# zhangyi-3/UCDIR

Measured on AMD Instinct MI355X. Metric: restored images/sec at 50-step p_sample_loop, 256x256 SID, higher is better.
Workload: dtype bf16

## Files before the change

ucdir_amd/csrc/engine.hip:

```cpp
#include <hip/hip_runtime.h>

#include <cmath>
#include <cstdio>
#include <cstring>
#include <map>
#include <mutex>
#include <set>
#include <array>
#include <atomic>
#include <memory>
#include <string>
#include <vector>

#include "../../include/ucdir_hip.h"
#include "cgemm.hip.h"
#include "conv_halo.hip.h"
#include "akgm_halo.hip.h"
#include "akgm_pre.hip.h"
#include "akgm_ws.hip.h"
#include "akgm_ws32.hip.h"
#include "akgm_ws64.hip.h"
#include "conv_ws.hip.h"
#include "conv_sk.hip.h"
#include "conv_ws128.hip.h"
#include "flash_attn2.hip.h"
#include "qkv_ws.hip.h"
#include "common.h"
#include "misc.hip.h"
#include "fewstep.hip.h"
#include "image_metrics.hip.h"
#include "pack.h"

static thread_local std::string g_err;
static int fail(const std::string& m) { g_err = m; return 1; }
#define HIPC(x)                                                                                   \
    do {                                                                                          \
        hipError_t e_ = (x);                                                                      \
        if (e_ != hipSuccess) {                                                                   \
            throw std::runtime_error(std::string(#x) + ": " + hipGetErrorString(e_));             \
        }                                                                                         \
    } while (0)
#define API_BEGIN try {
#define API_END                                                                                   \
    }                                                                                             \
    catch (const std::exception& e) { return fail(e.what()); }                                    \
    catch (...) { return fail("unknown error"); }                                                 \
    return 0;

static void require(bool c, const std::string& m) { if (!c) throw std::runtime_error(m); }

struct DevGuard {
    int prev = -1; bool changed = false;
    explicit DevGuard(int dev) {
        HIPC(hipGetDevice(&prev));
        if (prev != dev) { HIPC(hipSetDevice(dev)); changed = true; }
    }
    ~DevGuard() { if (changed) (void)hipSetDevice(prev); }
};

struct DevPool {
    std::vector<void*> ptrs;
    int64_t bytes = 0;
    void* alloc(size_t n, bool zero = true) {
        void* p = nullptr;
        if (n == 0) n = 16;
        HIPC(hipMalloc(&p, n));
        if (zero) HIPC(hipMemset(p, 0, n));
        ptrs.push_back(p); bytes += (int64_t)n;
        return p;
    }
    template <typename T> T* upload(const std::vector<T>& v) {
        T* p = (T*)alloc(v.size() * sizeof(T), false);
        if (!v.empty()) HIPC(hipMemcpy(p, v.data(), v.size() * sizeof(T), hipMemcpyHostToDevice));
        return p;
    }
    static constexpr size_t STAT_CAP = 1 << 21;
    stat_t* stat_slab = nullptr; size_t stat_used = 0;
    stat_t* alloc_stats(int B) {
        if (!stat_slab) stat_slab = (stat_t*)alloc(STAT_CAP * sizeof(stat_t), true);
        const size_t n = (size_t)2 * UCDIR_STAT_SLOTS * B;
        if (stat_used + n > STAT_CAP) throw std::runtime_error("DevPool: statistics slab exhausted");
        stat_t* p = stat_slab + stat_used; stat_used += n;
        return p;
    }
    void zero_stats(hipStream_t st) { if (stat_used) HIPC(hipMemsetAsync(stat_slab, 0, stat_used * sizeof(stat_t), st)); }
    void release() { for (void* p : ptrs) (void)hipFree(p); ptrs.clear(); bytes = 0; stat_slab = nullptr; stat_used = 0; }
    ~DevPool() { release(); }
};

struct ConvW {
    bf16_t* A = nullptr; float* bias = nullptr; float* Tb = nullptr; float* Tg = nullptr;
    int rows_pad = 0, Kpad = 0, ntaps = 0, cin = 0, cout = 0, TM = 128; bool fold = false;
    bf16_t* Aup = nullptr; int Kup = 0;
    bf16_t* A10 = nullptr; float* bias_res = nullptr;
    bf16_t* Aws = nullptr;
    bf16_t* Aws128 = nullptr;
    bf16_t* Aqkv = nullptr;
    bf16_t* Atile = nullptr;
    bf16_t* Ask[2] = {nullptr, nullptr}; bf16_t* Ask_up[2] = {nullptr, nullptr};
    long long sk_up_stride[2] = {0, 0};
    bf16_t* Ask1x1 = nullptr;
};
struct AkgmW {
    bf16_t* A = nullptr; float* bias = nullptr; float* Tb = nullptr; float* Tg = nullptr;
    float* Tbb = nullptr;
    bf16_t* Apre = nullptr;
    bf16_t* Aws32 = nullptr;
    bf16_t* Aws64 = nullptr;
    int C = 0, cg = 0, Kpad = 0;
};

static int pick_tm(int cout) { return cout >= 128 ? 128 : 64; }

static ConvW upload_conv(DevPool& pool, const float* w, const float* bias, const float* gamma, const float* beta,
                         int cout, int cin, int ks) {
    ConvW W;
    W.TM = pick_tm(cout);
    PackedConv P = pack_conv(w, bias, gamma, beta, cout, cin, ks, W.TM);
    W.A = pool.upload(P.A); W.bias = pool.upload(P.bias);
    W.fold = gamma != nullptr;
    if (W.fold) { W.Tb = pool.upload(P.Tb); W.Tg = pool.upload(P.Tg); }
    W.rows_pad = P.rows_pad; W.Kpad = P.Kpad; W.ntaps = P.ntaps; W.cin = cin; W.cout = cout;
    if (ks == 3 && cin == 64 && cout == 64 && P.Kpad == 576) W.Aws = pool.upload(pack_conv_ws(P));
    if (ks == 3 && cin % 32 == 0 && P.Kpad == 9 * cin && P.rows_pad % W.TM == 0) W.Atile = pool.upload(pack_conv_tiled(P, W.TM));
    if (ks == 3 && cin % 32 == 0 && P.Kpad == 9 * cin && cout % 128 == 0) {
        W.Ask[0] = pool.upload(pack_conv_sk(P.A, 1, P.rows_pad, P.Kpad, cin, 9, 1));
        if (cout % 256 == 0) W.Ask[1] = pool.upload(pack_conv_sk(P.A, 1, P.rows_pad, P.Kpad, cin, 9, 2));
    }
    if (ks == 1 && cin % 32 == 0 && P.Kpad == cin && cout % 128 == 0 && gamma == nullptr) W.Ask1x1 = pool.upload(pack_conv_sk(P.A, 1, P.rows_pad, P.Kpad, cin, 1, 1));
    if (ks == 1 && cout == 3 * cin && gamma != nullptr && (cin == 256 || cin == 512) && P.Kpad == cin && P.rows_pad >= cout) W.Aqkv = pool.upload(pack_qkv_ws(P, cin));
    return W;
}
static void upload_upconv(DevPool& pool, ConvW& W, const float* w, const float* bias) {
    PackedConv P = pack_upconv(w, bias, W.cout, W.cin, W.TM);
    W.Aup = pool.upload(P.A); W.Kup = P.Kpad;
    for (int mw = 1; mw <= 2; ++mw)
        if (W.cin % 32 == 0 && W.cout % (128 * mw) == 0) {
            std::vector<bf16_t> img = pack_conv_sk(P.A, 4, P.rows_pad, P.Kpad, W.cin, 4, mw);
            W.sk_up_stride[mw - 1] = (long long)((img.size() - (size_t)4 * 4 * mw * 2 * 512) / 4);
            W.Ask_up[mw - 1] = pool.upload(img);
        }
}
static AkgmW upload_akgm(DevPool& pool, const float* wsp, const float* bsp, const float* gamma, const float* beta, int C) {
    PackedAkgm P = pack_akgm(wsp, bsp, gamma, beta, C, 0);
    AkgmW W;
    W.A = pool.upload(P.A); W.bias = pool.upload(P.bias); W.Tb = pool.upload(P.Tb); W.Tg = pool.upload(P.Tg);
    W.C = C; W.cg = P.cg; W.Kpad = P.Kpad;
    {
        std::vector<float> tbb(P.Tb.size());
// ... 11 lines not shown
struct Profiler {
    bool on = false;
    std::vector<ProfEntry> entries;
    std::vector<hipEvent_t> pool; size_t used = 0;
    hipEvent_t get() {
        if (used == pool.size()) { hipEvent_t e; HIPC(hipEventCreate(&e)); pool.push_back(e); }
        return pool[used++];
    }
    ~Profiler() { for (auto e : pool) (void)hipEventDestroy(e); }
};
static Profiler g_prof;

template <int TM, int EPI, int MODE>
static void launch_one(const GemmP& p, dim3 grid, size_t lds, hipStream_t st) {
    hipLaunchKernelGGL((cgemm_kernel<TM, EPI, MODE>), grid, dim3(CG_THREADS), lds, st, p);
}

template <typename K> static void set_lds_attr(K* k, int bytes, bool abs0 = false) {
    HIPC(hipFuncSetAttribute((const void*)k, hipFuncAttributeMaxDynamicSharedMemorySize, bytes));
    if (abs0) {
        hipFuncAttributes fa;
        HIPC(hipFuncGetAttributes(&fa, (const void*)k));
        require(fa.sharedSizeBytes == 0, "a kernel with absolute LDS addressing has static __shared__ memory: its dynamic smem[] no longer starts at offset 0");
    }
}
template <int TM> static void set_cgemm_attrs() {
    set_lds_attr(cgemm_kernel<TM, EPI_STD, MODE_S1>, 100 * 1024, true); set_lds_attr(cgemm_kernel<TM, EPI_STD, MODE_DOWN>, 100 * 1024, true);
    set_lds_attr(cgemm_kernel<TM, EPI_STD, MODE_UP>, 100 * 1024, true); set_lds_attr(cgemm_kernel<TM, EPI_STD, MODE_PLAIN>, 100 * 1024, true);
    set_lds_attr(cgemm_kernel<TM, EPI_STD, MODE_S1C>, 100 * 1024, true); set_lds_attr(cgemm_kernel<TM, EPI_AKGM, MODE_S1>, 100 * 1024, true);
}
#define SPLITK_MAX_WGS 512
#define SK_MAX_GRID 256
#define SCRATCH_BYTES ((size_t)2 * SK_MAX_GRID * 65536 * sizeof(float))
static std::map<int, float*> g_splitk_buf;
static std::mutex g_static_mu;
static void ensure_kernel_attrs() {
    std::lock_guard<std::mutex> lk(g_static_mu);
    static std::set<int> done;
    int dev = 0;
    HIPC(hipGetDevice(&dev));
    if (done.count(dev)) return;
    set_cgemm_attrs<64>(); set_cgemm_attrs<128>();
    set_lds_attr(conv3x3_halo_kernel<128, false>, hc_lds_bytes<128>());
    set_lds_attr(conv3x3_halo_kernel<64, false>, hc_lds_bytes<64>());
    set_lds_attr(conv3x3_halo_kernel<64, true>, hc_lds_bytes<64>());
    set_lds_attr(akgm_halo_stage_kernel, AH_LDS); set_lds_attr(akgm_halo_kernel<true>, AH_LDS);
    set_lds_attr(akgm_pre_kernel<8>, AkPre<8>::LDS);
    set_lds_attr(akgm_ws_kernel<8>, AkWs::LDS); set_lds_attr(akgm_ws_kernel<16>, AkWs::LDS);
    set_lds_attr(akgm_ws32_kernel<32>, AkWs32::LDS); set_lds_attr(akgm_ws32_kernel<16>, AkWs32::LDS); set_lds_attr(akgm_ws32_kernel<8>, AkWs32::LDS);
    set_lds_attr(akgm_ws64_kernel<2, 8, true>, 160 * 1024); set_lds_attr(akgm_ws64_kernel<4, 8, true>, 160 * 1024);
    set_lds_attr(qkv_ws_kernel<256>, QkvWs::LDS); set_lds_attr(qkv_ws_kernel<512>, QkvWs::LDS);
    set_lds_attr(conv_ws_kernel, CvWs::LDS);
    set_lds_attr(conv_ws128_kernel, CvWs128::LDS);
    set_lds_attr(conv_sk_kernel<2, 8, 9>, 160 * 1024); set_lds_attr(conv_sk_kernel<2, 8, 4>, 160 * 1024);
    set_lds_attr(conv_sk_kernel<1, 8, 9>, 160 * 1024); set_lds_attr(conv_sk_kernel<1, 8, 4>, 160 * 1024);
    set_lds_attr(conv_sk_kernel<1, 4, 9>, 80 * 1024, true); set_lds_attr(conv_sk_kernel<1, 4, 4>, 80 * 1024, true);

    set_lds_attr(final_conv_kernel, 160 * 1024);
    set_lds_attr(flash_attn2_kernel<1, false>, fa_lds_bytes(128), true); set_lds_attr(flash_attn2_kernel<1, true>, fa_lds_bytes(128), true);
    set_lds_attr(flash_attn2_kernel<2, false>, fa_lds_bytes(256), true); set_lds_attr(flash_attn2_kernel<2, true>, fa_lds_bytes(256), true);
    set_lds_attr(flash_attn2_kernel<3, false>, fa_lds_bytes(384), true); set_lds_attr(flash_attn2_kernel<3, true>, fa_lds_bytes(384), true);
    set_lds_attr(flash_attn2_kernel<4, false>, fa_lds_bytes(512), true); set_lds_attr(flash_attn2_kernel<4, true>, fa_lds_bytes(512), true);
    done.insert(dev);
}

static void gemm_work(const GemmP& p, int epi, double& flops, double& bytes) {
    const double cols = ((p.cols_mode == COLS_PLAIN) ? (double)p.W : (double)p.H * p.W) * (p.up_phase ? 4.0 : 1.0);
    if (epi == EPI_AKGM) {
        const double C = 8.0 * p.cg;
        flops = 2.0 * 9 * C * C * cols * p.nbatch;
        bytes = (2.0 * C * cols * 2 + C * cols * 2 + cols * 32) * p.nbatch + 9.0 * C * C * 2;
    } else {
        const double K = (double)p.ntaps * p.cg;
        flops = 2.0 * K * p.nfeat * cols * p.nbatch;
        double in_cols = cols;
        if (p.cols_mode == COLS_DOWN) in_cols = cols * 4; else if (p.cols_mode == COLS_UP) in_cols = cols / 4;
        bytes = ((double)p.cg * in_cols * 2 + (double)p.nfeat * cols * (p.out_f32 ? 4 : 2) + (p.res ? (double)p.nfeat * cols * 2 : 0)) * p.nbatch
                + (p.a_bstride ? (double)p.nfeat * K * 2 * p.nbatch : (double)p.nfeat * K * 2);
    }
}

static void launch_cgemm_impl(const GemmP& p, int TM, int epi, hipStream_t st);
static void launch_cgemm(const GemmP& p, int TM, int epi, hipStream_t st) {
    if (!g_prof.on) { launch_cgemm_impl(p, TM, epi, st); return; }
    ProfEntry e;
    int mode = p.cols_mode; if (mode == COLS_S1 && p.in_compact) mode = MODE_S1C;
    e.key = (TM == 128 ? 100 : 0) + (epi == EPI_AKGM ? 10 : 0) + (epi == EPI_AKGM ? 0 : mode);
    gemm_work(p, epi, e.flops, e.bytes);
    e.dH = p.H; e.dW = p.W; e.dCin = p.cg * p.ntaps; e.dCout = p.nfeat;
    e.e0 = g_prof.get(); e.e1 = g_prof.get();
    HIPC(hipEventRecord(e.e0, st));
    launch_cgemm_impl(p, TM, epi, st);
    HIPC(hipEventRecord(e.e1, st));
    g_prof.entries.push_back(e);
}

static void launch_cgemm_impl(const GemmP& p0, int TM, int epi, hipStream_t st) {
    GemmP p = p0;
#ifdef UCDIR_TIMING
    static unsigned long long* cgdbg = nullptr;
    if (!cgdbg) HIPC(hipMalloc((void**)&cgdbg, 64 * 8));
    HIPC(hipMemsetAsync(cgdbg, 0, 64 * 8, st));
    p.dbg = cgdbg;
    struct Pr { unsigned long long* d; hipStream_t s; int mode, TM, nk; ~Pr() {
        unsigned long long h[64]; (void)hipStreamSynchronize(s); (void)hipMemcpy(h, d, sizeof(h), hipMemcpyDeviceToHost);
        const int n = (int)h[63]; fprintf(stderr, "CGEMM TIMING mode=%d TM=%d nk=%d n=%d:", mode, TM, nk, n);
// ... 364 lines not shown
    if (!dbgbuf) HIPC(hipMalloc((void**)&dbgbuf, 256 * 8));
    HIPC(hipMemset(dbgbuf, 0, 256 * 8));
    p.dbg = dbgbuf;
#endif
    int tm_run = w.TM;
    if (halo && tm_run == 128 && p.nbatch * p.tiles * p.rowtiles < 256) {
        tm_run = 64; p.rowtiles = w.rows_pad / 64;
    }
    static const bool fuse_res = !getenv("UCDIR_NO_FUSED_RES");
    bool did_res = false;
    if (halo && !upph && tm_run == 64 && w.TM == 64 && w.A10 && res_out && fuse_res) {
        p.A = w.A10; p.a_ld = 10 * cin; p.res_fused = 1; p.bias2 = w.bias_res;
        p.out2 = res_out->p; p.out2_bstride = res_out->bstride(); p.out2_ld = res_out->C;
        did_res = true;
    }
    const bool dual = did_res;
    static const bool use_atile = !getenv("UCDIR_NO_ATILE");
    if (use_atile && halo && !upph && !did_res && tm_run == w.TM && w.Atile && w.ntaps == 9) p.A_tiled = w.Atile;
    static const bool use_cws128 = !getenv("UCDIR_NO_CONV_WS128");
    if (use_cws128 && did_res && w.Aws128 && cin == 128 && x0.C == 64 && x1 && x1->C == 64 && !res && !p.out_nchw && y.H % 8 == 0 && y.W % 16 == 0 &&
        y.C == 64 && (g_persist_grid > 0 || (long long)y.B * (y.H / 8) * (y.W / 16) >= 4LL * num_cus())) {
        p.A = w.Aws128; p.alt_A = w.Aws128 + (size_t)2 * 72 * 2 * 32 * 8;
        p.th = 8; p.tw = 16; p.tiles_x = y.W / 16; p.tiles_y = y.H / 8;
        const int ntiles = y.B * p.tiles_x * p.tiles_y, ncu = num_cus();
        const int grid = ntiles < ncu ? ntiles : ncu;
#ifdef UCDIR_TIMING
        {
            static unsigned long long* dbgbuf = nullptr;
            if (!dbgbuf) HIPC(hipMalloc((void**)&dbgbuf, 256 * 8));
            HIPC(hipMemset(dbgbuf, 0, 256 * 8));
            p.dbg = dbgbuf;
            hipLaunchKernelGGL(conv_ws128_kernel, dim3(grid), dim3(CvWs128::THREADS), CvWs128::LDS, st, p);
            unsigned long long h[256];
            HIPC(hipStreamSynchronize(st));
            HIPC(hipMemcpy(h, dbgbuf, sizeof(h), hipMemcpyDeviceToHost));
            const int n = (int)h[255];
            fprintf(stderr, "CONV_WS128 TIMING n=%d:", n);
            for (int i = 1; i < n && i < 255; ++i) fprintf(stderr, " %llu", h[i] - h[i - 1]);
            fprintf(stderr, "\n");
            return did_res;
        }
#endif
        if (g_prof.on) {
            ProfEntry e; e.key = 24; gemm_work(p, EPI_STD, e.flops, e.bytes);
            { const double cols = (double)p.H * p.W * p.nbatch; e.flops += 2.0 * p.cg * p.nfeat * cols; e.bytes += 2.0 * p.cg * p.nfeat + 2.0 * p.nfeat * cols; }
            e.dH = p.H; e.dW = p.W; e.dCin = p.cg; e.dCout = p.nfeat;
            e.e0 = g_prof.get(); e.e1 = g_prof.get();
            HIPC(hipEventRecord(e.e0, st));
            hipLaunchKernelGGL(conv_ws128_kernel, dim3(grid), dim3(CvWs128::THREADS), CvWs128::LDS, st, p);
            HIPC(hipEventRecord(e.e1, st));
            g_prof.entries.push_back(e);
        } else {
            hipLaunchKernelGGL(conv_ws128_kernel, dim3(grid), dim3(CvWs128::THREADS), CvWs128::LDS, st, p);
        }
        HIPC(hipGetLastError());
        return did_res;
    }
    if (halo && !did_res && !p.out_nchw && w.cout % 8 == 0) {
        const int taps = upph ? 4 : 9, tps = 256 / tm_run;
        const int ks = choose_ksplit(p.nbatch * p.tiles * p.rowtiles, cin / HC_BK, (taps + tps - 1) / tps,
                                     (double)y.B * y.H * y.W * w.cout);
        if (ks > 1) { p.ksplit = ks; p.partial = splitk_scratch(); }
    }
    static const bool tail_res = !getenv("UCDIR_NO_TAIL_RES");
    if (halo && !upph && !did_res && res_out && wres && tail_res && !p.out_nchw && wres->ntaps == 1 &&
        wres->rows_pad >= p.rowtiles * tm_run) {
        p.alt_blocks = p.nbatch * p.tiles * p.rowtiles;
        p.alt_A = wres->A; p.alt_a_ld = wres->Kpad; p.bias2 = wres->bias;
        p.out2 = res_out->p; p.out2_bstride = res_out->bstride(); p.out2_ld = res_out->C;
        did_res = true;
    }
    static const bool use_cws = !getenv("UCDIR_NO_CONV_WS");
    if (use_cws && halo && !upph && !did_res && !dual && w.Aws && !x1 && !res && !p.out_nchw && p.ksplit <= 1 && !p.alt_blocks &&
        y.H % 16 == 0 && y.W % 16 == 0 && x0.C == 64 && y.C == 64 &&
        (g_persist_grid > 0 || (long long)y.B * (y.H / 16) * (y.W / 16) >= 4LL * num_cus())) {
        p.A = w.Aws; p.th = 16; p.tw = 16; p.tiles_x = y.W / 16; p.tiles_y = y.H / 16;
        const int ntiles = y.B * p.tiles_x * p.tiles_y, ncu = num_cus();
        const int grid = ntiles < ncu ? ntiles : ncu;
#ifdef UCDIR_TIMING
        {
            static unsigned long long* dbgbuf = nullptr;
            if (!dbgbuf) HIPC(hipMalloc((void**)&dbgbuf, 512 * 8));
            HIPC(hipMemset(dbgbuf, 0, 512 * 8));
            p.dbg = dbgbuf;
            hipLaunchKernelGGL(conv_ws_kernel, dim3(grid), dim3(HC_THREADS), CvWs::LDS, st, p);
            unsigned long long h[512];
            HIPC(hipStreamSynchronize(st));
            HIPC(hipMemcpy(h, dbgbuf, sizeof(h), hipMemcpyDeviceToHost));
            for (int w = 0; w < 2; ++w) {
                const int n = (int)h[w * 256 + 255];
                fprintf(stderr, "CONV_WS TIMING %s n=%d:", w ? "late" : "early", n);
                for (int i = 1; i < n && i < 255; ++i) fprintf(stderr, " %llu", h[w * 256 + i] - h[w * 256 + i - 1]);
                fprintf(stderr, "\n");
            }
            return did_res;
        }
#endif
        if (g_prof.on) {
            ProfEntry e; e.key = 23; gemm_work(p, EPI_STD, e.flops, e.bytes);
            e.dH = p.H; e.dW = p.W; e.dCin = p.cg; e.dCout = p.nfeat;
            e.e0 = g_prof.get(); e.e1 = g_prof.get();
            HIPC(hipEventRecord(e.e0, st));
            hipLaunchKernelGGL(conv_ws_kernel, dim3(grid), dim3(HC_THREADS), CvWs::LDS, st, p);
            HIPC(hipEventRecord(e.e1, st));
            g_prof.entries.push_back(e);
        } else {
// ... 479 lines not shown
}

static const std::vector<float>& W_(ucdir_ctx* c, const std::string& name, size_t expect) {
    auto it = c->host.find(name);
    require(it != c->host.end(), "missing weight: " + name);
    require(it->second.v.size() == expect, "weight " + name + " has wrong size");
    return it->second.v;
}

static void finalize_weights(ucdir_ctx* c) {
    const auto& cfg = c->cfg;
    const int inner = cfg.inner_channel;
    c->wpool.release();
    c->lw.assign(c->layers.size(), LayerW());
    c->mlp_w1 = c->wpool.upload(W_(c, "noise_level_mlp.1.weight", (size_t)4 * inner * inner));
    c->mlp_b1 = c->wpool.upload(W_(c, "noise_level_mlp.1.bias", (size_t)4 * inner));
    c->mlp_w2 = c->wpool.upload(W_(c, "noise_level_mlp.3.weight", (size_t)4 * inner * inner));
    c->mlp_b2 = c->wpool.upload(W_(c, "noise_level_mlp.3.bias", (size_t)inner));
    std::vector<float> tw;
    int nb = 0;
    for (size_t li = 0; li < c->layers.size(); ++li) {
        const LayerDesc& d = c->layers[li];
        LayerW& w = c->lw[li];
        if (d.kind == "stem") {
            const auto& sw = W_(c, d.name + ".weight", (size_t)d.cout * d.cin * 9);
            require(d.cin == 6, "stem expects in_channel == 6 (cat[cond, x_t])");
            std::vector<float> t((size_t)54 * d.cout);
            for (int o = 0; o < d.cout; ++o) for (int ci = 0; ci < 6; ++ci) for (int k = 0; k < 9; ++k)
                t[(size_t)(k * 6 + ci) * d.cout + o] = sw[((size_t)o * 6 + ci) * 9 + k];
            require(d.cout % 64 == 0, "stem: inner_channel must be a multiple of 64");
            w.stem_w = c->wpool.upload(pack_stem_frags(t, W_(c, d.name + ".bias", (size_t)d.cout), 6, d.cout));
        } else if (d.kind == "down" || d.kind == "up") {
            w.conv = upload_conv(c->wpool, W_(c, d.name + ".conv.weight", (size_t)d.cout * d.cin * 9).data(),
                                 W_(c, d.name + ".conv.bias", d.cout).data(), nullptr, nullptr, d.cout, d.cin, 3);
            if (d.kind == "up") upload_upconv(c->wpool, w.conv, W_(c, d.name + ".conv.weight", (size_t)d.cout * d.cin * 9).data(),
                                              W_(c, d.name + ".conv.bias", d.cout).data());
        } else {
            const std::string r = d.name + ".res_block.";
            w.block_index = nb++;
            w.conv = upload_conv(c->wpool, W_(c, r + "conv1.weight", (size_t)d.cout * d.cin * 9).data(),
                                 W_(c, r + "conv1.bias", d.cout).data(), W_(c, r + "norm1.weight", d.cin).data(),
                                 W_(c, r + "norm1.bias", d.cin).data(), d.cout, d.cin, 3);
            w.has_res = d.cin != d.cout;
            if (w.has_res) {
                w.resconv = upload_conv(c->wpool, W_(c, r + "res_conv.weight", (size_t)d.cout * d.cin).data(),
                                        W_(c, r + "res_conv.bias", d.cout).data(), nullptr, nullptr, d.cout, d.cin, 1);
                if (w.conv.TM == 64 && d.cin % 64 == 0 && w.conv.Kpad == 9 * d.cin) {
                    PackedConv P = pack_conv(W_(c, r + "conv1.weight", (size_t)d.cout * d.cin * 9).data(), nullptr,
                                             W_(c, r + "norm1.weight", d.cin).data(), W_(c, r + "norm1.bias", d.cin).data(),
                                             d.cout, d.cin, 3, 64);
                    const std::vector<bf16_t> a10 = pack_conv_res10(P, W_(c, r + "res_conv.weight", (size_t)d.cout * d.cin).data());
                    w.conv.A10 = c->wpool.upload(a10);
                    if (d.cin == 128 && d.cout == 64) w.conv.Aws128 = c->wpool.upload(pack_conv_ws128(a10));
                    w.conv.bias_res = w.resconv.bias;
                }
            }
            w.sp = upload_akgm(c->wpool, W_(c, r + "spdyconv.weight", (size_t)8 * d.cout * (d.cout / 8) * 9).data(),
                               W_(c, r + "spdyconv.bias", (size_t)8 * d.cout).data(), W_(c, r + "norm2.weight", d.cout).data(),
                               W_(c, r + "norm2.bias", d.cout).data(), d.cout);
            std::vector<float> gw;
            for (const char* s : {"conv2.0.weight", "conv2.0.bias", "conv2.2.weight", "conv2.2.bias"}) {
                const auto& v = c->host.at(r + s).v;
                gw.insert(gw.end(), v.begin(), v.end());
            }
            require(gw.size() == 48 + 16 + 576 + 8, "guide branch weights have wrong size");
            w.gw = c->wpool.upload(gw);
            for (const char* s : {"noise_func.0.weight", "noise_func.0.bias", "noise_func.2.weight", "noise_func.2.bias"}) {
                const auto& v = c->host.at(r + s).v;
                tw.insert(tw.end(), v.begin(), v.end());
            }
            if (d.attn) {
                const std::string a = d.name + ".attn.";
                const std::vector<float> wf = fold_out_into_v(W_(c, a + "qkv.weight", (size_t)3 * d.cout * d.cout).data(),
                                                              W_(c, a + "out.weight", (size_t)d.cout * d.cout).data(), d.cout);
                w.qkv = upload_conv(c->wpool, wf.data(), nullptr,
                                    W_(c, a + "norm.weight", d.cout).data(), W_(c, a + "norm.bias", d.cout).data(),
                                    3 * d.cout, d.cout, 1);
                w.outp = upload_conv(c->wpool, W_(c, a + "out.weight", (size_t)d.cout * d.cout).data(),
                                     W_(c, a + "out.bias", d.cout).data(), nullptr, nullptr, d.cout, d.cout, 1);
            }
        }
    }
    c->nblocks = nb;
    require(tw.size() == (size_t)nb * (8 * inner + 8 + 64 + 8), "time weights have wrong size");
    c->tw = c->wpool.upload(tw);
    const int fc = inner * cfg.channel_mults[0];
    c->fin_gamma = c->wpool.upload(W_(c, "final_conv.0.weight", fc));
    c->fin_beta = c->wpool.upload(W_(c, "final_conv.0.bias", fc));
    c->fin_conv = upload_conv(c->wpool, W_(c, "final_conv.3.weight", (size_t)cfg.out_channel * fc * 9).data(),
                              W_(c, "final_conv.3.bias", cfg.out_channel).data(), nullptr, nullptr, cfg.out_channel, fc, 3);
    if (cfg.out_channel <= 4 && fc % 32 == 0) {
        c->fin_w = c->wpool.upload(pack_final_frags(W_(c, "final_conv.3.weight", (size_t)cfg.out_channel * fc * 9).data(), cfg.out_channel, fc));
        c->fin_b = c->wpool.upload(W_(c, "final_conv.3.bias", cfg.out_channel));
    }
    c->host.clear();
    c->finalized = true;
}

static int level_dim(int d, int level) { return d >> level; }

struct ActPlanner {
    DevPool& pool; int B; bool reuse;
    std::map<std::array<int, 3>, std::vector<bf16_t*>> free_;
    Act get(int h, int w, int C, bool stats = true) {
        Act a; a.B = B; a.H = h; a.W = w; a.C = C;
        auto& fl = free_[{h, w, C}];
// ... 581 lines not shown
}

int32_t ucdir_op_conv(const float* x0, int32_t c0, const float* x1, int32_t c1, int32_t B, int32_t H, int32_t W,
                      const float* w_host, const float* bias_host, const float* gamma_host, const float* beta_host,
                      int32_t cout, int32_t ksize, int32_t mode, int32_t silu, const float* residual, float* y,
                      double* stats_out_host, void* stream) {
    API_BEGIN
    ensure_kernel_attrs();
    hipStream_t st = (hipStream_t)stream;
    DevPool pool;
    Act a0 = act_from_nchw(pool, x0, B, c0, H, W, st, true);
    Act a1; if (x1) a1 = act_from_nchw(pool, x1, B, c1, H, W, st, true);
    int Ho = H, Wo = W;
    if (mode == COLS_DOWN) { Ho = H / 2; Wo = W / 2; } else if (mode == COLS_UP) { Ho = 2 * H; Wo = 2 * W; }
    Act out = make_act(pool, B, Ho, Wo, cout);
    Act res; if (residual) res = act_from_nchw(pool, residual, B, cout, Ho, Wo, st, false);
    ConvW w = upload_conv(pool, w_host, bias_host, gamma_host, beta_host, cout, c0 + (x1 ? c1 : 0), ksize);
    if (mode == COLS_UP && ksize == 3) upload_upconv(pool, w, w_host, bias_host);
    run_conv(w, a0, x1 ? &a1 : nullptr, out, mode, silu, residual ? &res : nullptr, true, st);
    hipLaunchKernelGGL(act_to_nchw_kernel, dim3(2048), dim3(256), 0, st, out.p, y, B, cout, Ho, Wo);
    HIPC(hipGetLastError());
    std::vector<stat_t> sfx;
    if (stats_out_host) { sfx.resize((size_t)2 * UCDIR_STAT_SLOTS * B); HIPC(hipMemcpyAsync(sfx.data(), out.stats, sizeof(stat_t) * sfx.size(), hipMemcpyDeviceToHost, st)); }
    HIPC(hipStreamSynchronize(st));
    if (stats_out_host)
        for (int bb = 0; bb < B; ++bb)
            for (int q = 0; q < 2; ++q) {
                stat_t acc = 0;
                for (int k = 0; k < UCDIR_STAT_SLOTS; ++k) acc += sfx[((size_t)bb * UCDIR_STAT_SLOTS + k) * 2 + q];
                stats_out_host[bb * 2 + q] = (double)acc / UCDIR_STAT_SCALE;
            }
    API_END
}

int32_t ucdir_op_conv_res(const float* x0, int32_t c0, const float* x1, int32_t c1, int32_t B, int32_t H, int32_t W,
                          const float* w_host, const float* bias_host, const float* gamma_host, const float* beta_host,
                          const float* wres_host, const float* bres_host, int32_t cout, int32_t silu,
                          float* y, float* yres, double* stats_out_host, void* stream) {
    API_BEGIN
    ensure_kernel_attrs();
    hipStream_t st = (hipStream_t)stream;
    DevPool pool;
    const int cin = c0 + (x1 ? c1 : 0);
    Act a0 = act_from_nchw(pool, x0, B, c0, H, W, st, true);
    Act a1; if (x1) a1 = act_from_nchw(pool, x1, B, c1, H, W, st, true);
    Act out = make_act(pool, B, H, W, cout), rout = make_act(pool, B, H, W, cout, false);
    ConvW w = upload_conv(pool, w_host, bias_host, gamma_host, beta_host, cout, cin, 3);
    ConvW wr = upload_conv(pool, wres_host, bres_host, nullptr, nullptr, cout, cin, 1);
    if (w.TM == 64 && cin % 64 == 0 && w.Kpad == 9 * cin) {
        PackedConv P = pack_conv(w_host, nullptr, gamma_host, beta_host, cout, cin, 3, 64);
        const std::vector<bf16_t> a10 = pack_conv_res10(P, wres_host);
        w.A10 = pool.upload(a10); w.bias_res = wr.bias;
        if (cin == 128 && cout == 64) w.Aws128 = pool.upload(pack_conv_ws128(a10));
    }
    const bool did = run_conv(w, a0, x1 ? &a1 : nullptr, out, COLS_S1, silu, nullptr, true, st, nullptr, 0, 0, &rout, &wr);
    if (!did) run_conv(wr, a0, x1 ? &a1 : nullptr, rout, COLS_S1, 0, nullptr, false, st);
    hipLaunchKernelGGL(act_to_nchw_kernel, dim3(2048), dim3(256), 0, st, out.p, y, B, cout, H, W);
    hipLaunchKernelGGL(act_to_nchw_kernel, dim3(2048), dim3(256), 0, st, rout.p, yres, B, cout, H, W);
    HIPC(hipGetLastError());
    std::vector<stat_t> sfx;
    if (stats_out_host) { sfx.resize((size_t)2 * UCDIR_STAT_SLOTS * B); HIPC(hipMemcpyAsync(sfx.data(), out.stats, sizeof(stat_t) * sfx.size(), hipMemcpyDeviceToHost, st)); }
    HIPC(hipStreamSynchronize(st));
    if (stats_out_host)
        for (int bb = 0; bb < B; ++bb)
            for (int q = 0; q < 2; ++q) {
                stat_t acc = 0;
                for (int k = 0; k < UCDIR_STAT_SLOTS; ++k) acc += sfx[((size_t)bb * UCDIR_STAT_SLOTS + k) * 2 + q];
                stats_out_host[bb * 2 + q] = (double)acc / UCDIR_STAT_SCALE;
            }
    API_END
}

int32_t ucdir_op_akgm(const float* h, const float* att, const float* res, int32_t B, int32_t C, int32_t H, int32_t W,
                      const float* wsp_host, const float* bsp_host, const float* gamma_host, const float* beta_host,
                      float* y, double* stats_out_host, void* stream) {
    API_BEGIN
    ensure_kernel_attrs();
    hipStream_t st = (hipStream_t)stream;
    DevPool pool;
    Act ah = act_from_nchw(pool, h, B, C, H, W, st, true);
    Act ar = act_from_nchw(pool, res, B, C, H, W, st, false);
    Act out = make_act(pool, B, H, W, C);
    float* G = (float*)pool.alloc((size_t)B * H * W * 8 * 4);
    hipLaunchKernelGGL(nchw8_to_compact_kernel, dim3(1024), dim3(256), 0, st, att, G, B, H, W);
    std::vector<float> ones((size_t)B * 8, 1.f);
    float* attw = pool.upload(ones);
    AkgmW w = upload_akgm(pool, wsp_host, bsp_host, gamma_host, beta_host, C);
    float* tcbuf = (float*)pool.alloc((size_t)B * (9 * 8 * C + 2) * sizeof(float), false);
    run_akgm(w, ah, G, attw, ar, out, tcbuf, st);
    hipLaunchKernelGGL(act_to_nchw_kernel, dim3(2048), dim3(256), 0, st, out.p, y, B, C, H, W);
    HIPC(hipGetLastError());
    std::vector<stat_t> sfx;
    if (stats_out_host) { sfx.resize((size_t)2 * UCDIR_STAT_SLOTS * B); HIPC(hipMemcpyAsync(sfx.data(), out.stats, sizeof(stat_t) * sfx.size(), hipMemcpyDeviceToHost, st)); }
    HIPC(hipStreamSynchronize(st));
    if (stats_out_host)
        for (int bb = 0; bb < B; ++bb)
            for (int q = 0; q < 2; ++q) {
                stat_t acc = 0;
                for (int k = 0; k < UCDIR_STAT_SLOTS; ++k) acc += sfx[((size_t)bb * UCDIR_STAT_SLOTS + k) * 2 + q];
                stats_out_host[bb * 2 + q] = (double)acc / UCDIR_STAT_SCALE;
            }
    API_END
}

int32_t ucdir_op_attention(const float* x, int32_t B, int32_t C, int32_t H, int32_t W, const float* gamma_host,
                           const float* beta_host, const float* wqkv_host, const float* wout_host, const float* bout_host,
// ... 265 lines not shown
```

ucdir_amd/csrc/pack.h:

```cpp
#pragma once
#include <cmath>
#include <cstdint>
#include <vector>

#include "common.h"

struct PackedConv {
    std::vector<bf16_t> A;
    std::vector<float> bias;
    std::vector<float> Tb, Tg;
    int rows_pad = 0, Kpad = 0, ntaps = 0, cin = 0, cout = 0, ncls = 0;
};

static inline bool tap_valid(int cls, int tap) {
    const int cy = cls / 3, cx = cls % 3, ky = tap / 3, kx = tap % 3;
    if (cy == 0 && ky == 0) return false;
    if (cy == 2 && ky == 2) return false;
    if (cx == 0 && kx == 0) return false;
    if (cx == 2 && kx == 2) return false;
    return true;
}

static inline PackedConv pack_conv(const float* w, const float* bias, const float* gamma, const float* beta,
                                   int cout, int cin, int ks, int TM) {
// ... 14 lines not shown
                const float ws = fold ? wv * gamma[c] : wv;
                const bf16_t q = f2bf(ws);
                P.A[(size_t)o * P.Kpad + (size_t)t * cin + c] = q;
                if (fold) {
                    wb[(size_t)t * cout + o] += (double)wv * beta[c];
                    wg[(size_t)t * cout + o] += (double)bf2f(q);
                }
            }
    if (fold) {
        P.Tb.assign((size_t)P.ncls * cout, 0.f);
        P.Tg.assign((size_t)P.ncls * cout, 0.f);
        for (int cls = 0; cls < P.ncls; ++cls)
            for (int o = 0; o < cout; ++o) {
                double sb = 0, sg = 0;
                for (int t = 0; t < P.ntaps; ++t) {
                    const int t9 = (P.ntaps == 9) ? t : 4;
                    if (P.ncls == 9 && !tap_valid(cls, t9)) continue;
                    sb += wb[(size_t)t * cout + o]; sg += wg[(size_t)t * cout + o];
                }
                P.Tb[(size_t)cls * cout + o] = (float)sb;
                P.Tg[(size_t)cls * cout + o] = (float)sg;
            }
    }
    return P;
}

static inline std::vector<bf16_t> pack_conv_ws(const PackedConv& P) {
    std::vector<bf16_t> img((size_t)2 * 36 * 2 * 32 * 8, 0);
    for (int rw = 0; rw < 2; ++rw)
        for (int j = 0; j < 36; ++j)
            for (int hk = 0; hk < 2; ++hk)
                for (int rho = 0; rho < 32; ++rho) {
                    const int o = 32 * rw + 16 * ((rho >> 2) & 1) + (rho & 3) + 4 * (rho >> 3);
                    const int tap = j >> 2, c0 = 16 * (j & 3) + 8 * hk;
                    for (int e = 0; e < 8; ++e)
                        img[((((size_t)rw * 36 + j) * 2 + hk) * 32 + rho) * 8 + e] = P.A[(size_t)o * P.Kpad + (size_t)tap * 64 + c0 + e];
                }
    return img;
}

static inline std::vector<bf16_t> pack_conv_ws128(const std::vector<bf16_t>& A10) {
    const int K10 = 10 * 128, nj = 80;
    std::vector<bf16_t> img((size_t)2 * nj * 2 * 32 * 8, 0);
    for (int rw = 0; rw < 2; ++rw)
        for (int j = 0; j < nj; ++j)
            for (int hk = 0; hk < 2; ++hk)
                for (int rho = 0; rho < 32; ++rho) {
                    const int o = 32 * rw + 16 * ((rho >> 2) & 1) + (rho & 3) + 4 * (rho >> 3);
                    const int tap = j >> 3, c0 = 16 * (j & 7) + 8 * hk;
                    const size_t dst = j < 72 ? ((((size_t)rw * 72 + j) * 2 + hk) * 32 + rho) * 8
                                              : (size_t)2 * 72 * 2 * 32 * 8 + ((((size_t)rw * 8 + (j - 72)) * 2 + hk) * 32 + rho) * 8;
                    for (int e = 0; e < 8; ++e) img[dst + e] = A10[(size_t)o * K10 + (size_t)tap * 128 + c0 + e];
                }
    return img;
}

static inline std::vector<bf16_t> pack_conv_res10(const PackedConv& P, const float* wres) {
    const int cin = P.cin, K10 = 10 * cin;
    std::vector<bf16_t> A((size_t)P.rows_pad * K10, 0);
    for (int o = 0; o < P.rows_pad; ++o) {
        for (int k = 0; k < 9 * cin; ++k) A[(size_t)o * K10 + k] = P.A[(size_t)o * P.Kpad + k];
        if (o < P.cout)
            for (int c = 0; c < cin; ++c) A[(size_t)o * K10 + 9 * cin + c] = f2bf(wres[(size_t)o * cin + c]);
    }
    return A;
}

struct PackedAkgm {
    std::vector<bf16_t> A;
    std::vector<float> bias;
    std::vector<float> Tb, Tg;
    int C = 0, cg = 0, Kpad = 0;
};

static inline PackedAkgm pack_akgm(const float* wsp, const float* bsp, const float* gamma, const float* beta, int C,
                                   int kpad_override = 0) {
    PackedAkgm P;
    P.C = C; P.cg = C / 8;
    const int cg = P.cg;
    const bool chunked = (cg == 64) && !kpad_override;
    P.Kpad = kpad_override ? kpad_override : (chunked ? 640 : ((9 * cg + 63) / 64) * 64);
    P.A.assign((size_t)8 * C * P.Kpad, 0);
    P.bias.assign((size_t)8 * C, 0.f);
    P.Tb.assign((size_t)9 * 8 * C, 0.f);
    P.Tg.assign((size_t)9 * 8 * C, 0.f);
    for (int o = 0; o < 8 * C; ++o) P.bias[o] = bsp[o];
    for (int g = 0; g < 8; ++g)
        for (int pr = 0; pr < C; ++pr) {
            const int t32 = pr / 32, rho = pr % 32;
            const int floc = 4 * t32 + ((rho >> 4) & 1) * 2 + ((rho >> 2) & 1);
            const int s = (rho & 3) + 4 * ((rho >> 3) & 1);
            const int o = g * C + 8 * floc + s;
            bf16_t* row = &P.A[((size_t)g * C + pr) * P.Kpad];
            double wb[9] = {0}, wg[9] = {0};
            for (int ci = 0; ci < cg; ++ci) {
                const int cglob = g * cg + ci;
                for (int t = 0; t < 9; ++t) {
                    const float wv = wsp[((size_t)o * cg + ci) * 9 + t];
                    const bf16_t q = f2bf(wv * gamma[cglob]);
                    row[chunked ? (size_t)(ci / 32) * 320 + (size_t)t * 32 + (ci % 32) : (size_t)t * cg + ci] = q;
                    wb[t] += (double)wv * beta[cglob];
                    wg[t] += (double)bf2f(q);
                }
            }
            for (int cls = 0; cls < 9; ++cls) {
                double sb = 0, sg = 0;
// ... 178 lines not shown
```

Baseline: 37.00.

## Add persistent weight-stationary conv kernel for 192-to-64 residual blocks

Adds a specialized persistent weight-stationary 3x3 conv kernel for cin=192 (128+64 concatenated inputs), cout=64. It also fuses the 1x1 residual conv. Weights are held in registers, and a double-buffered halo is staged in LDS. The K dimension is split across wave pairs, and the partial sums are exchanged through LDS. It replaces the generic path for these decoder blocks. The cost is heavy register pressure from the 60 weight fragments held per lane, plus new packing code.

After: 37.25 (median of 6 runs). Within noise of the previous version (+0.7%).

```diff
diff --git a/ucdir_amd/csrc/conv_ws192.hip.h b/ucdir_amd/csrc/conv_ws192.hip.h
--- /dev/null
+++ b/ucdir_amd/csrc/conv_ws192.hip.h
@@ -0,0 +1,297 @@
+#pragma once
+#include <type_traits>
+#include "conv_ws128.hip.h"
+
+struct CvWs192 {
+    static constexpr int TH = 4, TW = 16;
+    static constexpr int PITCH = 24;
+    static constexpr int PLANE = 6 * PITCH * 128;
+    static constexpr int HALO = 3 * PLANE;
+    static constexpr int QSTEP = 2 * PITCH * 128;
+    static constexpr int OFF_X = 2 * HALO;
+    static constexpr int X_WAVE = 8 * 64 * 16;
+    static constexpr int OFF_TCS = OFF_X + 4 * X_WAVE;
+    static constexpr int OFF_B2 = OFF_TCS + 9 * 64 * 4;
+    static constexpr int OFF_SCAL = OFF_B2 + 64 * 4;
+    static constexpr int LDS = OFF_SCAL + 128;
+    static constexpr int THREADS = 256;
+    static constexpr int DEPTH = 3;
+    static constexpr int NJ = 54;
+};
+
+__global__ __launch_bounds__(CvWs192::THREADS, 1) void conv_ws192_kernel(const GemmP p) {
+    using L = CvWs192;
+    extern __shared__ __attribute__((aligned(16))) unsigned char smem[];
+    float* const tcs = reinterpret_cast<float*>(smem + L::OFF_TCS);
+    float* const b2s = reinterpret_cast<float*>(smem + L::OFF_B2);
+    float* const scal = reinterpret_cast<float*>(smem + L::OFF_SCAL);
+    const int tid = threadIdx.x, lane = tid & 63, l31 = lane & 31, hh = lane >> 5;
+    const int wave = __builtin_amdgcn_readfirstlane(tid >> 6);
+    const int rw = wave & 1, kh = wave >> 1;
+    const int prow = l31 >> 4, pcol = (l31 & 15) ^ (prow << 3);
+    int lid;
+    {
+        const int nblk = gridDim.x, bid = blockIdx.x;
+        const int q = nblk >> 3, r = nblk & 7, xcd = bid & 7;
+        lid = (xcd < r ? xcd * (q + 1) : r * (q + 1) + (xcd - r) * q) + (bid >> 3);
+    }
+#ifdef UCDIR_TIMING
+    const bool dbg_on = p.dbg && (lid == (int)gridDim.x / 2 + 3) && (lane == 0) && (wave == 1);
+    int dbg_n = 0;
+#define C9_STAMP() do { if (dbg_on && dbg_n < 250) p.dbg[dbg_n++] = __builtin_amdgcn_s_memtime(); } while (0)
+#else
+#define C9_STAMP() do {} while (0)
+#endif
+    C9_STAMP();
+    const int tps = p.tiles_x * p.tiles_y;
+    const int T = p.nbatch * tps;
+    const int t_beg = (int)((long long)lid * T / (int)gridDim.x), t_end = (int)((long long)(lid + 1) * T / (int)gridDim.x);
+    if (t_beg >= t_end) return;
+
+    bf16x8_t af[L::NJ], ra[6];
+    {
+        const bf16_t* Ab = p.A + ((((rw * 2 + kh) * (L::NJ + 6)) * 2 + hh) * 32 + l31) * 8;
+#pragma unroll
+        for (int j = 0; j < L::NJ; ++j) af[j] = *reinterpret_cast<const bf16x8_t*>(Ab + j * (2 * 32 * 8));
+#pragma unroll
+        for (int j = 0; j < 6; ++j) ra[j] = *reinterpret_cast<const bf16x8_t*>(Ab + (L::NJ + j) * (2 * 32 * 8));
+    }
+#pragma unroll
+    for (int j = 0; j < L::NJ; ++j) asm volatile("" : "+v"(af[j]));
+#pragma unroll
+    for (int j = 0; j < 6; ++j) asm volatile("" : "+v"(ra[j]));
+    if (tid < 64) b2s[tid] = p.bias2 ? p.bias2[tid] : 0.f;
+    __syncthreads();
+
+    const int nunits = wave < 2 ? 5 : 4;
+    unsigned hrel[5][3];
+#pragma unroll
+    for (int s = 0; s < 5; ++s) {
+        const int u = wave + 4 * s, r = u / 3, pl = u - 3 * r;
+        const int C = pl == 2 ? 64 : 128, chb = pl == 1 ? 64 : 0;
+#pragma unroll
+        for (int c3 = 0; c3 < 3; ++c3) {
+            const int col = c3 * 8 + (lane >> 3), gcol = col < 18 ? col : 17, hp = r * L::PITCH + col;
+            hrel[s][c3] = (unsigned)((r * p.Wp + gcol) * C + chb + (((lane & 7) ^ ((hp >> 1) & 7)) << 3)) * 2u;
+        }
+    }
+    auto issue_piece = [&](const unsigned char* h0, const unsigned char* h1, unsigned char* hd, int s, int c3) {
+        const int u = wave + 4 * s, r = u / 3, pl = u - 3 * r;
+        stage16(reinterpret_cast<const bf16_t*>((pl == 2 ? h1 : h0) + hrel[s][c3]), hd + pl * L::PLANE + (3 * r + c3) * 1024, lane);
+    };
+    unsigned ba[3][4], bb[3][2][2];
+    {
+        const int hp0 = prow * L::PITCH + pcol;
+#pragma unroll
+        for (int kx = 0; kx < 3; ++kx) {
+            const int sxh = (((hp0 + kx) >> 1) & 7) ^ hh;
+#pragma unroll
+            for (int k2 = 0; k2 < 4; ++k2) ba[kx][k2] = kh * 2 * L::PLANE + ((hp0 + kx) << 7) + (((2 * k2) ^ sxh) << 4);
+#pragma unroll
+            for (int c = 0; c < 2; ++c)
+#pragma unroll
+                for (int f = 0; f < 2; ++f)
+                    bb[kx][c][f] = L::PLANE + ((hp0 + kx) << 7) + (((2 * ((2 * kh + c) ^ (2 * f))) ^ sxh) << 4);
+        }
+    }
+    const unsigned tc_lane = L::OFF_TCS + (32 * rw + 16 * hh) * 4;
+    const unsigned b2_lane = L::OFF_B2 + (32 * rw + 16 * hh) * 4;
+    const unsigned x_put = L::OFF_X + (rw * 2 + kh) * L::X_WAVE + lane * 16;
+    const unsigned x_get = L::OFF_X + (rw * 2 + (kh ^ 1)) * L::X_WAVE + lane * 16;
+    const unsigned rel_out = (unsigned)(((2 * kh + prow + 1) * p.Wp + pcol + 1) * 64 + 32 * rw + 16 * hh) * 2;
+
+    int b, ty, tx;
+    {
+        b = t_beg / tps;
+        const int r = t_beg - b * tps;
+        ty = r / p.tiles_x; tx = r - ty * p.tiles_x;
+    }
+    auto tile_src = [&](int nb, int nty, int ntx, const unsigned char*& h0, const unsigned char*& h1) {
+        const long long pix0 = (long long)nty * L::TH * p.Wp + ntx * L::TW;
+        h0 = reinterpret_cast<const unsigned char*>(p.B0 + (long long)nb * p.b0_bstride + pix0 * 128);
+        h1 = reinterpret_cast<const unsigned char*>(p.B1 + (long long)nb * p.b1_bstride + pix0 * 64);
+    };
+    {
+        const unsigned char *h0, *h1;
+        tile_src(b, ty, tx, h0, h1);
+#pragma unroll
+        for (int s = 0; s < 5; ++s)
+            if (s < nunits)
+#pragma unroll
+                for (int c3 = 0; c3 < 3; ++c3) issue_piece(h0, h1, smem, s, c3);
+    }
+
+    int b_cur = -1;
+    float rstd_a = 1.f;
+    stat_t S1 = 0, S2 = 0;
+    const int act = p.act;
+
+#pragma unroll 1
+    for (int t = t_beg; t < t_end; ++t) {
+        const int buf = (t - t_beg) & 1;
+        const bool last = t + 1 == t_end;
+        C9_STAMP();
+        if (t == t_beg) { HC_WAIT(0); }
+        asm volatile("s_barrier" ::: "memory");
+        C9_STAMP();
+        if (b != b_cur) {
+            if (b_cur >= 0 && p.stats_out) {
+                const stat_t a = wave_sum_ll(S1), q2 = wave_sum_ll(S2);
+                if (lane == 0) stat_add_fx(p.stats_out, b_cur, a, q2);
+            }
+            S1 = 0; S2 = 0;
+            b_cur = b;
+            if (wave == 0) {
+                float mean = 0.f, rstd = 1.f;
+                if (p.fold) {
+                    long long v = 0;
+                    if (lane < 2 * UCDIR_STAT_SLOTS) {
+                        v = p.stats0[(long long)b * (2 * UCDIR_STAT_SLOTS) + lane];
+                        if (p.stats1) v += p.stats1[(long long)b * (2 * UCDIR_STAT_SLOTS) + lane];
+                    }
+#pragma unroll
+                    for (int off = 2; off < 2 * UCDIR_STAT_SLOTS; off <<= 1) v += __shfl_xor(v, off);
+                    const long long q = __shfl(v, 1);
+                    mean_rstd(stat_val(v), stat_val(q), p.inv_count, mean, rstd);
+                }
+                if (lane == 0) { scal[0] = mean; scal[1] = rstd; }
+            }
+            __syncthreads();
+            const float mean = scal[0], rstd = scal[1];
+            for (int i = tid; i < 9 * 64; i += L::THREADS) {
+                const int cls = i >> 6, f = i & 63;
+                float v = p.bias ? p.bias[f] : 0.f;
+                if (p.fold) v += p.Tb[(long long)cls * p.tab_ld + f] - mean * rstd * p.Tg[(long long)cls * p.tab_ld + f];
+                tcs[i] = v;
+            }
+            rstd_a = __builtin_bit_cast(float, __builtin_amdgcn_readfirstlane(__builtin_bit_cast(int, p.alpha * (p.fold ? rstd : 1.0f))));
+            __syncthreads();
+        }
+        int nb = b, nty = ty, ntx = tx + 1;
+        if (ntx == p.tiles_x) { ntx = 0; if (++nty == p.tiles_y) { nty = 0; ++nb; } }
+
+        if (t != t_beg) {
+            const int d = buf ? L::HALO : -L::HALO;
+#pragma unroll
+            for (int kx = 0; kx < 3; ++kx) {
+#pragma unroll
+                for (int k2 = 0; k2 < 4; ++k2) ba[kx][k2] += d;
+#pragma unroll
+                for (int c = 0; c < 2; ++c) { bb[kx][c][0] += d; bb[kx][c][1] += d; }
+            }
+        }
+
+        f32x16_t acc[2], acc2[2];
+        {
+            bf16x8_t bq[L::DEPTH + 1][2];
+            const unsigned char *h0, *h1;
+            tile_src(nb, nty, ntx, h0, h1);
+            unsigned char* const hd = smem + (buf ^ 1) * L::HALO;
+            auto read_step = [&](auto jc, bf16x8_t (&dst)[2]) {
+                constexpr int j = decltype(jc)::value;
+                constexpr int tap = j / 6, cl = j % 6, ky = tap / 3, kx = tap - 3 * ky;
+                constexpr int off = ky * (L::PITCH * 128);
+                if constexpr (cl < 4) {
+                    lds_read16_asm<off>(dst[0], ba[kx][cl ^ (ky == 1 ? 2 : 0)]);
+                    lds_read16_asm<off + L::QSTEP>(dst[1], ba[kx][cl ^ (ky == 1 ? 2 : 0)]);
+                } else {
+                    lds_read16_asm<off>(dst[0], bb[kx][cl & 1][ky == 1 ? 1 : 0]);
+                    lds_read16_asm<off + L::QSTEP>(dst[1], bb[kx][cl & 1][ky == 1 ? 1 : 0]);
+                }
+            };
+            __builtin_amdgcn_sched_barrier(0);
+            asm volatile("s_waitcnt lgkmcnt(0)" ::: "memory");
+            static_for<0, L::DEPTH>([&](auto jc) { read_step(jc, bq[decltype(jc)::value]); });
+            static_for<0, L::NJ>([&](auto jc) {
+                constexpr int j = decltype(jc)::value;
+                if constexpr (j + L::DEPTH < L::NJ)
+                    read_step(std::integral_constant<int, j + L::DEPTH>{}, bq[(j + L::DEPTH) % (L::DEPTH + 1)]);
+                if constexpr (j % 3 == 1 && j / 3 < 15) {
+                    constexpr int e = j / 3, s = e / 3, c3 = e % 3;
+                    if (!last && s < nunits) issue_piece(h0, h1, hd, s, c3);
+                }
+                constexpr int ahead = (L::NJ - 1 - j) < L::DEPTH ? (L::NJ - 1 - j) : L::DEPTH;
+                lgkm_wait_asm<2 * ahead>();
+                const f32x16_t zero = {0.f, 0.f, 0.f, 0.f, 0.f, 0.f, 0.f, 0.f, 0.f, 0.f, 0.f, 0.f, 0.f, 0.f, 0.f, 0.f};
+                const bf16x8_t* bj = bq[j % (L::DEPTH + 1)];
+                acc[0] = __builtin_amdgcn_mfma_f32_32x32x16_bf16(af[j], bj[0], j ? acc[0] : zero, 0, 0, 0);
+                acc[1] = __builtin_amdgcn_mfma_f32_32x32x16_bf16(af[j], bj[1], j ? acc[1] : zero, 0, 0, 0);
+                if constexpr (j / 6 == 4) {
+                    constexpr int cl = j % 6;
+                    acc2[0] = __builtin_amdgcn_mfma_f32_32x32x16_bf16(ra[cl], bj[0], cl ? acc2[0] : zero, 0, 0, 0);
+                    acc2[1] = __builtin_amdgcn_mfma_f32_32x32x16_bf16(ra[cl], bj[1], cl ? acc2[1] : zero, 0, 0, 0);
+                }
+            });
+            __builtin_amdgcn_sched_barrier(0);
+        }
+        C9_STAMP();
+        f32x16_t own, own2;
+        {
+            const f32x16_t give = kh ? acc[0] : acc[1], give2 = kh ? acc2[0] : acc2[1];
+            own = kh ? acc[1] : acc[0]; own2 = kh ? acc2[1] : acc2[0];
+#pragma unroll
+            for (int g = 0; g < 4; ++g) {
+                const f32x4_t v = {give[4 * g], give[4 * g + 1], give[4 * g + 2], give[4 * g + 3]};
+                const f32x4_t w = {give2[4 * g], give2[4 * g + 1], give2[4 * g + 2], give2[4 * g + 3]};
+                *reinterpret_cast<f32x4_t*>(smem + x_put + 1024 * g) = v;
+                *reinterpret_cast<f32x4_t*>(smem + x_put + 1024 * (4 + g)) = w;
+            }
+        }
+        asm volatile("s_waitcnt lgkmcnt(0)\n\ts_barrier" ::: "memory");
+        C9_STAMP();
+        const bool interior = ty > 0 && tx > 0 && ty + 1 < p.tiles_y && tx + 1 < p.tiles_x;
+        const long long tile_el = (long long)(ty * L::TH * p.Wp + tx * L::TW) * 64;
+        unsigned char* outb = reinterpret_cast<unsigned char*>(reinterpret_cast<bf16_t*>(p.out) + (long long)b * p.out_bstride + tile_el);
+        unsigned char* out2b = reinterpret_cast<unsigned char*>(p.out2 + (long long)b * p.out2_bstride + tile_el);
+        float s1 = 0.f, s2 = 0.f;
+        uint4 pk[2], pk2[2];
+        {
+            unsigned tca = tc_lane + 4 * 256;
+            if (!interior) {
+                const int r = 2 * kh + prow, c = pcol;
+                const int cy = (ty == 0 && r == 0) ? 0 : ((ty + 1 == p.tiles_y && r == L::TH - 1) ? 2 : 1);
+                const int cx = (tx == 0 && c == 0) ? 0 : ((tx + 1 == p.tiles_x && c == L::TW - 1) ? 2 : 1);
+                tca = tc_lane + (cy * 3 + cx) * 256;
+            }
+            float v[16], w[16];
+#pragma unroll
+            for (int g = 0; g < 4; ++g) {
+                const f32x4_t o4 = *reinterpret_cast<const f32x4_t*>(smem + x_get + 1024 * g);
+                const f32x4_t o24 = *reinterpret_cast<const f32x4_t*>(smem + x_get + 1024 * (4 + g));
+                const f32x4_t c4 = *reinterpret_cast<const f32x4_t*>(smem + tca + 16 * g);
+                const f32x4_t d4 = *reinterpret_cast<const f32x4_t*>(smem + b2_lane + 16 * g);
+#pragma unroll
+                for (int e = 0; e < 4; ++e) {
+                    v[4 * g + e] = fmaf(own[4 * g + e] + o4[e], rstd_a, c4[e]);
+                    w[4 * g + e] = (own2[4 * g + e] + o24[e]) + d4[e];
+                }
+            }
+            if (act == 1) {
+#pragma unroll
+                for (int i = 0; i < 16; ++i) v[i] = silu_fast(v[i]);
+            } else if (act == 2) {
+#pragma unroll
+                for (int i = 0; i < 16; ++i) v[i] = fmaxf(0.2f * v[i], v[i]);
+            }
+#pragma unroll
+            for (int i = 0; i < 16; ++i) { s1 += v[i]; s2 += v[i] * v[i]; }
+            pk[0] = pack8_bf16(v); pk[1] = pack8_bf16(v + 8);
+            pk2[0] = pack8_bf16(w); pk2[1] = pack8_bf16(w + 8);
+        }
+        C9_STAMP();
+        HC_WAIT(0);
+        *reinterpret_cast<uint4*>(outb + rel_out) = pk[0];
+        *reinterpret_cast<uint4*>(outb + rel_out + 16) = pk[1];
+        *reinterpret_cast<uint4*>(out2b + rel_out) = pk2[0];
+        *reinterpret_cast<uint4*>(out2b + rel_out + 16) = pk2[1];
+        S1 += stat_fx((double)s1); S2 += stat_fx((double)s2);
+        b = nb; ty = nty; tx = ntx;
+    }
+#ifdef UCDIR_TIMING
+    if (dbg_on) p.dbg[255] = dbg_n;
+#endif
+    if (p.stats_out) {
+        const stat_t a = wave_sum_ll(S1), q2 = wave_sum_ll(S2);
+        if (lane == 0) stat_add_fx(p.stats_out, b_cur, a, q2);
+    }
+}
diff --git a/ucdir_amd/csrc/engine.hip b/ucdir_amd/csrc/engine.hip
--- a/ucdir_amd/csrc/engine.hip
+++ b/ucdir_amd/csrc/engine.hip
@@ -23,6 +23,7 @@
 #include "conv_ws.hip.h"
 #include "conv_sk.hip.h"
 #include "conv_ws128.hip.h"
+#include "conv_ws192.hip.h"
 #include "flash_attn2.hip.h"
 #include "qkv_ws.hip.h"
 #include "common.h"
@@ -95,6 +96,7 @@
     bf16_t* A10 = nullptr; float* bias_res = nullptr;
     bf16_t* Aws = nullptr;
     bf16_t* Aws128 = nullptr;
+    bf16_t* Aws192 = nullptr;
     bf16_t* Aqkv = nullptr;
     bf16_t* Atile = nullptr;
     bf16_t* Ask[2] = {nullptr, nullptr}; bf16_t* Ask_up[2] = {nullptr, nullptr};
@@ -212,6 +214,7 @@
     set_lds_attr(qkv_ws_kernel<256>, QkvWs::LDS); set_lds_attr(qkv_ws_kernel<512>, QkvWs::LDS);
     set_lds_attr(conv_ws_kernel, CvWs::LDS);
     set_lds_attr(conv_ws128_kernel, CvWs128::LDS);
+    set_lds_attr(conv_ws192_kernel, CvWs192::LDS);
     set_lds_attr(conv_sk_kernel<2, 8, 9>, 160 * 1024); set_lds_attr(conv_sk_kernel<2, 8, 4>, 160 * 1024);
     set_lds_attr(conv_sk_kernel<1, 8, 9>, 160 * 1024); set_lds_attr(conv_sk_kernel<1, 8, 4>, 160 * 1024);
     set_lds_attr(conv_sk_kernel<1, 4, 9>, 80 * 1024, true); set_lds_attr(conv_sk_kernel<1, 4, 4>, 80 * 1024, true);
@@ -682,6 +685,45 @@
             g_prof.entries.push_back(e);
         } else {
             hipLaunchKernelGGL(conv_ws128_kernel, dim3(grid), dim3(CvWs128::THREADS), CvWs128::LDS, st, p);
+        }
+        HIPC(hipGetLastError());
+        return did_res;
+    }
+    if (use_cws128 && did_res && w.Aws192 && cin == 192 && x0.C == 128 && x1 && x1->C == 64 && !res && !p.out_nchw &&
+        y.H % CvWs192::TH == 0 && y.W % CvWs192::TW == 0 && y.C == 64 &&
+        (g_persist_grid > 0 || (long long)y.B * (y.H / CvWs192::TH) * (y.W / CvWs192::TW) >= 4LL * num_cus())) {
+        p.A = w.Aws192;
+        p.th = CvWs192::TH; p.tw = CvWs192::TW; p.tiles_x = y.W / CvWs192::TW; p.tiles_y = y.H / CvWs192::TH;
+        const int ntiles = y.B * p.tiles_x * p.tiles_y;
+        const int grid = ntiles < num_cus() ? ntiles : num_cus();
+#ifdef UCDIR_TIMING
+        {
+            static unsigned long long* dbgbuf = nullptr;
+            if (!dbgbuf) HIPC(hipMalloc((void**)&dbgbuf, 256 * 8));
+            HIPC(hipMemset(dbgbuf, 0, 256 * 8));
+            p.dbg = dbgbuf;
+            hipLaunchKernelGGL(conv_ws192_kernel, dim3(grid), dim3(CvWs192::THREADS), CvWs192::LDS, st, p);
+            unsigned long long h[256];
+            HIPC(hipStreamSynchronize(st));
+            HIPC(hipMemcpy(h, dbgbuf, sizeof(h), hipMemcpyDeviceToHost));
+            const int n = (int)h[255];
+            fprintf(stderr, "CONV_WS192 TIMING n=%d:", n);
+            for (int i = 1; i < n && i < 255; ++i) fprintf(stderr, " %llu", h[i] - h[i - 1]);
+            fprintf(stderr, "\n");
+            return did_res;
+        }
+#endif
+        if (g_prof.on) {
+            ProfEntry e; e.key = 26; gemm_work(p, EPI_STD, e.flops, e.bytes);
+            { const double cols = (double)p.H * p.W * p.nbatch; e.flops += 2.0 * p.cg * p.nfeat * cols; e.bytes += 2.0 * p.cg * p.nfeat + 2.0 * p.nfeat * cols; }
+            e.dH = p.H; e.dW = p.W; e.dCin = p.cg; e.dCout = p.nfeat;
+            e.e0 = g_prof.get(); e.e1 = g_prof.get();
+            HIPC(hipEventRecord(e.e0, st));
+            hipLaunchKernelGGL(conv_ws192_kernel, dim3(grid), dim3(CvWs192::THREADS), CvWs192::LDS, st, p);
+            HIPC(hipEventRecord(e.e1, st));
+            g_prof.entries.push_back(e);
+        } else {
+            hipLaunchKernelGGL(conv_ws192_kernel, dim3(grid), dim3(CvWs192::THREADS), CvWs192::LDS, st, p);
         }
         HIPC(hipGetLastError());
         return did_res;
@@ -1267,6 +1309,7 @@
                     const std::vector<bf16_t> a10 = pack_conv_res10(P, W_(c, r + "res_conv.weight", (size_t)d.cout * d.cin).data());
                     w.conv.A10 = c->wpool.upload(a10);
                     if (d.cin == 128 && d.cout == 64) w.conv.Aws128 = c->wpool.upload(pack_conv_ws128(a10));
+                    if (d.cin == 192 && d.cout == 64) w.conv.Aws192 = c->wpool.upload(pack_conv_ws192(a10));
                     w.conv.bias_res = w.resconv.bias;
                 }
             }
@@ -1954,6 +1997,7 @@
         const std::vector<bf16_t> a10 = pack_conv_res10(P, wres_host);
         w.A10 = pool.upload(a10); w.bias_res = wr.bias;
         if (cin == 128 && cout == 64) w.Aws128 = pool.upload(pack_conv_ws128(a10));
+        if (cin == 192 && cout == 64) w.Aws192 = pool.upload(pack_conv_ws192(a10));
     }
     const bool did = run_conv(w, a0, x1 ? &a1 : nullptr, out, COLS_S1, silu, nullptr, true, st, nullptr, 0, 0, &rout, &wr);
     if (!did) run_conv(wr, a0, x1 ? &a1 : nullptr, rout, COLS_S1, 0, nullptr, false, st);
diff --git a/ucdir_amd/csrc/pack.h b/ucdir_amd/csrc/pack.h
--- a/ucdir_amd/csrc/pack.h
+++ b/ucdir_amd/csrc/pack.h
@@ -90,6 +90,23 @@
                                               : (size_t)2 * 72 * 2 * 32 * 8 + ((((size_t)rw * 8 + (j - 72)) * 2 + hk) * 32 + rho) * 8;
                     for (int e = 0; e < 8; ++e) img[dst + e] = A10[(size_t)o * K10 + (size_t)tap * 128 + c0 + e];
                 }
+    return img;
+}
+
+static inline std::vector<bf16_t> pack_conv_ws192(const std::vector<bf16_t>& A10) {
+    const int cin = 192, K10 = 10 * cin, nj = 60;
+    std::vector<bf16_t> img((size_t)2 * 2 * nj * 2 * 32 * 8, 0);
+    for (int rw = 0; rw < 2; ++rw)
+        for (int kh = 0; kh < 2; ++kh)
+            for (int j = 0; j < nj; ++j)
+                for (int hk = 0; hk < 2; ++hk)
+                    for (int rho = 0; rho < 32; ++rho) {
+                        const int o = 32 * rw + 16 * ((rho >> 2) & 1) + (rho & 3) + 4 * (rho >> 3);
+                        const int tap = j < 54 ? j / 6 : 9, cl = j < 54 ? j % 6 : j - 54;
+                        const int c0 = (kh == 0 ? 16 * cl : (cl < 4 ? 128 + 16 * cl : 96 + 16 * (cl - 4))) + 8 * hk;
+                        const size_t dst = (((((size_t)rw * 2 + kh) * nj + j) * 2 + hk) * 32 + rho) * 8;
+                        for (int e = 0; e < 8; ++e) img[dst + e] = A10[(size_t)o * K10 + (size_t)tap * cin + c0 + e];
+                    }
     return img;
 }
 
```
